# maxjiang93/space_time_pde

Hardware: AMD Instinct MI355X
Metric: query-points/sec (fwd+PDE-residual bwd), rb2d 128^3 latent (higher is better)
Workload: dtype f32; 1 GPU; BASELINE configs[1]: latent [1,32,128,128,32], 2^20 query points, RB2 (3 transport + continuity), ImNet nf=32 softplus, L1 losses, backward to ImNet + UNet3d parameters; points=1048576, parallelism=points sharded x1, unet=UNet3d(igres=(32, 128, 128), nf=16, mf=256) fwd+bwd inside the timed step

## Files before the change

include/stpde_hip.h:

```cpp
#ifndef STPDE_HIP_H
#define STPDE_HIP_H

#ifdef __cplusplus
extern "C" {
#endif

#define STPDE_OK 0
#define STPDE_E_BADARG 1
#define STPDE_E_UNSUPPORTED 2
#define STPDE_E_LAUNCH 3

#define STPDE_ACT_TANH 0
#define STPDE_ACT_RELU 1
#define STPDE_ACT_SOFTPLUS 2
#define STPDE_ACT_ELU 3
#define STPDE_ACT_SWISH 4
#define STPDE_ACT_LEAKYRELU 5

#define STPDE_XT 3
#define STPDE_PBAR_SLOTS 64

typedef struct {
  int S1;
  int S2;
// ... 2 lines not shown
  int act;
  float act_param;
  int combo;
  float alpha[6];
} stpde_jet_cfg;

int stpde_version(void);
int stpde_last_error(char* buf, unsigned long n);
#define STPDE_TUNE_CONV3_LDS_OFF 0
#define STPDE_TUNE_CONV3_LDS_MINBLK 1
#define STPDE_TUNE_CONV3_LDS_GX 2
#define STPDE_TUNE_CONV_WGRAD_LDS_GX 3
#define STPDE_TUNE_CONV1_WGRAD_LDS_GX 4
#define STPDE_TUNE_WGRAD_FP32_SWAP 5
#define STPDE_TUNE_FC2_BWD_FUSED 6
#define STPDE_TUNE_COUNT 7
int stpde_tune(const char* name, int value);
int stpde_trace_enable(int on);
long stpde_trace_read(char* buf, unsigned long n);

typedef struct {
  int P, N, B, n0, n1, n2, C;
  int p_base;
  float lo_c[3], hi_c[3], cube[3];
  float alpha[6];
} stpde_gather_desc;
int stpde_lig_gather(const stpde_gather_desc* d, const float* pts, const float* latent, float* X, float* XR,
                     float* coef, int* cell, float* cw , void* stream);

typedef struct {
  int ntiles, KT, MT, first_hidden;
// ... 30 lines not shown

int stpde_jet_layer_bwd_to(const stpde_layer_desc* d, const float* abar_out, const float* WhT_pack, const float* in_pre,
                           float* abar_in, const float* cw, float* act_param_bar, const void* WhT_pack_bf16, void* stream);

int stpde_jet_wgrad(const stpde_layer_desc* d, int SP, const float* abar_out, const float* in_pre, const float* X,
                    const float* tanc0, float* dW_aug, const float* cw, void* stream);

int stpde_jet_fc1_bwd_supported(const stpde_layer_desc* d);
int stpde_jet_fc1_bwd(const stpde_layer_desc* d, const float* abar1, const void* WhT_pack_bf16, const float* z0,
                      const float* tanc0, const float* cw, const float* X, float* abar0, float* abar0_tan, float* dW_aug,
                      float* act_param_bar, void* stream);

int stpde_jet_fc2_bwd_supported(const stpde_layer_desc* d);
int stpde_jet_fc2_bwd(const stpde_layer_desc* d, const float* abar2, const float* WhT_pack, const float* pre1, const float* X,
                      const float* cw, float* abar1, float* dW_aug, float* act_param_bar, void* stream);

int stpde_lig_reduce_fwd(const stpde_jet_cfg* cfg, int S_mlp, int P, int n_out, const float* out_pre,
                         const float* coef, float* jets, long ldp, void* stream);
int stpde_lig_reduce_bwd(const stpde_jet_cfg* cfg, int S_mlp, int P, int n_out, const float* jets_bar, long ldp,
                         const float* coef, float* abar_out, void* stream);

int stpde_jet_tan0_reduce(int ntiles, int MT, const float* abar0_tan, float* dW_aug, int ldw, int det ,
                          void* stream);

typedef struct {
  int ntiles, nlayers, C, n1, n2;
  int MT[8];
  int SP[8];
  int packed[8];
  int S[8];
// ... 40 lines not shown
  unsigned long sort_tmp_bytes;
  float* abar4x;
} stpde_lig_workspace;
#define STPDE_F_STASH 1
#define STPDE_F_VALUE_TILES 2
#define STPDE_F_FUSED_TAIL 4
#define STPDE_F_TAN0_ROWSUM 8
#define STPDE_F_DETERMINISTIC 16
#define STPDE_F_WGRAD 32
#define STPDE_F_WGRAD_FP32 64
#define STPDE_F_PHASE_A 128
#define STPDE_F_PHASE_B 256
#define STPDE_F_NO_FC1_FUSED 512
#define STPDE_F_DET 1024
#define STPDE_F_FC2_FUSED 2048
int stpde_lig_imnet_jet_fwd(const stpde_imnet_plan* plan, const stpde_jet_cfg* cfg_mlp, const stpde_jet_cfg* cfg_out,
                            const stpde_gather_desc* gd, const float* pts, const float* latent,
                            const stpde_lig_workspace* ws, float* jets, long ldp, int flags, void* stream);
int stpde_lig_imnet_jet_bwd(const stpde_imnet_plan* plan, const stpde_jet_cfg* cfg_mlp, const stpde_jet_cfg* cfg_out,
                            const stpde_jet_cfg* cfg_val, const stpde_gather_desc* gd, const stpde_lig_workspace* ws,
                            const float* jets_bar, long ldp, float* dW_flat, float* dlatent, float* act_param_bar,
                            int flags, void* stream);
unsigned long stpde_lig_sort_tmp_bytes(int P, long n_nodes);
int stpde_lig_cell_sort(int P, long n_nodes, const int* cell, int* perm, int* start, void* tmp, unsigned long tmp_bytes,
                        void* stream);

typedef struct {
  int P, N, B, dim, C;
  int n[4];
  float lo_c[4], hi_c[4], cube[4];
// ... 256 lines not shown
```

space_time_pde_amd/_lib.py:

```python
import ctypes as C
import os
import subprocess
import threading

_HERE = os.path.dirname(os.path.abspath(__file__))
_CSRC = os.path.join(_HERE, "csrc")
LIB_PATH = os.environ.get("STPDE_LIB") or os.path.join(_HERE, "libstpde_hip.so")
_SOURCES = ["jet_layer.hip", "jet_layer_s00.hip", "jet_layer_s03.hip", "jet_layer_s30.hip", "jet_layer_s31.hip", "jet_layer_s32.hip", "jet_layer_s34.hip", "jet_layer_s36.hip", "jet_tail.hip", "jet_wgrad.hip", "jet_wgrad_s00.hip", "jet_wgrad_s30.hip", "jet_wgrad_s31.hip", "jet_wgrad_s32.hip", "jet_wgrad_s34.hip", "jet_wgrad_s36.hip", "jet_fc1_bwd.hip", "jet_fc2_bwd.hip", "lig_gather_reduce.hip", "lig_pipeline.hip", "interp_nd.hip", "conv3d.hip", "conv3d_fused.hip", "optim.hip", "residual.hip", "bn.hip", "resample.hip", "sampler.hip", "sampler_median.hip", "api.cpp"]
_HIPFLAGS = ["--offload-arch=gfx950", "-O3", "-std=c++17", "-fPIC", "-ffp-contract=off", "-munsafe-fp-atomics",
             "--offload-compress"]

ABI_VERSION = 316

ACT_CODES = {"tanh": 0, "relu": 1, "softplus": 2, "elu": 3, "swish": 4, "leakyrelu": 5}
PBAR_SLOTS = 64
XT = 3


class JetCfg(C.Structure):
    _fields_ = [("S1", C.c_int), ("S2", C.c_int), ("pair0", C.c_int * 6), ("pair1", C.c_int * 6),
                ("act", C.c_int), ("act_param", C.c_float), ("combo", C.c_int), ("alpha", C.c_float * 6)]


class GatherDesc(C.Structure):
# ... 21 lines not shown
class ImNetPlanDesc(C.Structure):
    _fields_ = [("nlayers", C.c_int), ("cin", C.c_int), ("cout", C.c_int), ("nf16", C.c_int), ("KT", C.c_int * 8),
                ("MT", C.c_int * 8), ("Wh", C.c_void_p * 8), ("WhT", C.c_void_p * 8), ("Ws", C.c_void_p * 8),
                ("WsL", C.c_void_p * 8), ("tanc", C.c_void_p * 8), ("Wh16", C.c_void_p * 8), ("WhT16", C.c_void_p * 8),
                ("mfma_bf16", C.c_int), ("packed_mask", C.c_int), ("dw_off", C.c_long * 8)]


class LigWorkspace(C.Structure):
    _fields_ = [("X", C.c_void_p), ("XR", C.c_void_p), ("coef", C.c_void_p), ("cw", C.c_void_p), ("cell", C.c_void_p),
                ("pre", C.c_void_p * 8), ("abar2x", C.c_void_p), ("abar3x", C.c_void_p), ("tan0", C.c_void_p),
                ("abar0", C.c_void_p), ("abar1x", C.c_void_p), ("abar0x", C.c_void_p), ("xrows", C.c_void_p), ("perm", C.c_void_p), ("start", C.c_void_p),
                ("sort_tmp", C.c_void_p), ("sort_tmp_bytes", C.c_ulong), ("abar4x", C.c_void_p)]


F_STASH, F_VALUE_TILES, F_FUSED_TAIL, F_TAN0_ROWSUM, F_DETERMINISTIC, F_WGRAD, F_WGRAD_FP32 = 1, 2, 4, 8, 16, 32, 64
F_PHASE_A, F_PHASE_B, F_NO_FC1_FUSED, F_DET, F_FC2_FUSED = 128, 256, 512, 1024, 2048
LOSS_DET = 16


class Conv3dDesc(C.Structure):
    _fields_ = [("B", C.c_int), ("T", C.c_int), ("Z", C.c_int), ("X", C.c_int), ("Ci", C.c_int), ("Co", C.c_int),
                ("ksize", C.c_int), ("det", C.c_int), ("mfma_bf16", C.c_int)]


class Conv3dFusedArgs(C.Structure):
    _fields_ = [("d", Conv3dDesc), ("x", C.c_void_p), ("w_pack", C.c_void_p), ("bias", C.c_void_p), ("y", C.c_void_p),
                ("x2", C.c_void_p), ("w2_pack", C.c_void_p), ("y2", C.c_void_p), ("wo2_pack", C.c_void_p),
                ("bias2", C.c_void_p), ("in_sums", C.c_void_p), ("in_gamma", C.c_void_p), ("in_beta", C.c_void_p),
                ("in_running_mean", C.c_void_p), ("in_running_var", C.c_void_p), ("in_stat", C.c_void_p),
                ("out_sums", C.c_void_p), ("m", C.c_void_p), ("m_stat", C.c_void_p), ("m_gamma", C.c_void_p),
                ("m_beta", C.c_void_p), ("m_bsum", C.c_void_p), ("Ci2", C.c_int), ("Co2", C.c_int),
# ... 173 lines not shown
    "stpde_jet_layer_bwd_to": ([C.POINTER(LayerDesc)] + [_VP] * 8, C.c_int),
    "stpde_jet_tail_fwd": ([C.POINTER(JetCfg), C.c_int, C.c_int, _VP, _VP, C.POINTER(_VP), C.POINTER(_VP), C.POINTER(_VP),
                            C.POINTER(_VP), _VP, _VP], C.c_int),
    "stpde_jet_tail_bwd": ([C.POINTER(JetCfg), C.c_int, C.c_int, _VP, C.POINTER(_VP), C.POINTER(_VP), C.POINTER(_VP), _VP,
                            _VP, _VP], C.c_int),
    "stpde_jet_tail_fwd_p": ([C.POINTER(JetCfg), C.c_int, C.c_int, _VP, _VP, C.POINTER(_VP), C.POINTER(_VP), C.POINTER(_VP),
                              C.POINTER(_VP), _VP, C.c_int, C.POINTER(_VP), _VP], C.c_int),
    "stpde_jet_tail_bwd_p": ([C.POINTER(JetCfg), C.c_int, C.c_int, _VP, C.POINTER(_VP), C.POINTER(_VP), C.POINTER(_VP), _VP,
                              _VP, C.c_int, C.POINTER(_VP), _VP], C.c_int),
    "stpde_jet_tan0_reduce": ([C.c_int, C.c_int, _VP, _VP, C.c_int, C.c_int, _VP], C.c_int),
    "stpde_jet_wgrad": ([C.POINTER(LayerDesc), C.c_int] + [_VP] * 7, C.c_int),
    "stpde_jet_fc1_bwd_supported": ([C.POINTER(LayerDesc)], C.c_int),
    "stpde_jet_fc1_bwd": ([C.POINTER(LayerDesc)] + [_VP] * 11, C.c_int),
    "stpde_jet_fc2_bwd_supported": ([C.POINTER(LayerDesc)], C.c_int),
    "stpde_jet_fc2_bwd": ([C.POINTER(LayerDesc)] + [_VP] * 9, C.c_int),
    "stpde_lig_reduce_fwd": ([C.POINTER(JetCfg), C.c_int, C.c_int, C.c_int, _VP, _VP, _VP, C.c_long, _VP], C.c_int),
    "stpde_lig_reduce_bwd": ([C.POINTER(JetCfg), C.c_int, C.c_int, C.c_int, _VP, C.c_long, _VP, _VP, _VP], C.c_int),
    "stpde_lig_xbar_scatter": ([C.POINTER(XbarDesc), C.POINTER(_VP), C.POINTER(_VP), _VP, _VP, _VP], C.c_int),
    "stpde_lig_xbar_rows": ([C.POINTER(XbarDesc), C.POINTER(_VP), C.POINTER(_VP), _VP, _VP], C.c_int),
    "stpde_lig_dlatent_reduce": ([C.c_int] * 5 + [_VP] * 5, C.c_int),
    "stpde_lig_imnet_jet_fwd": ([C.POINTER(ImNetPlanDesc), C.POINTER(JetCfg), C.POINTER(JetCfg), C.POINTER(GatherDesc), _VP,
                                 _VP, C.POINTER(LigWorkspace), _VP, C.c_long, C.c_int, _VP], C.c_int),
    "stpde_lig_imnet_jet_bwd": ([C.POINTER(ImNetPlanDesc), C.POINTER(JetCfg), C.POINTER(JetCfg), C.POINTER(JetCfg),
                                 C.POINTER(GatherDesc), C.POINTER(LigWorkspace), _VP, C.c_long, _VP, _VP, _VP, C.c_int, _VP],
                                C.c_int),
    "stpde_lig_sort_tmp_bytes": ([C.c_int, C.c_long], C.c_ulong),
    "stpde_lig_cell_sort": ([C.c_int, C.c_long, _VP, _VP, _VP, _VP, C.c_ulong, _VP], C.c_int),
    "stpde_interp_fwd": ([C.POINTER(InterpDesc)] + [_VP] * 7, C.c_int),
    "stpde_interp_bwd_grid": ([C.POINTER(InterpDesc)] + [_VP] * 5, C.c_int),
    "stpde_conv3d_fwd": ([C.POINTER(Conv3dDesc)] + [_VP] * 5, C.c_int),
# ... 170 lines not shown
```

space_time_pde_amd/csrc/api.cpp:

```cpp
#include <hip/hip_runtime.h>

#include <cstdarg>
#include <cstdio>
#include <cstring>
#include <mutex>
#include <set>
#include <string>

#include "../../include/stpde_hip.h"

static thread_local char g_err[512] = "";

void stpde_set_error(const char* fmt, ...) {
  va_list ap;
  va_start(ap, fmt);
  vsnprintf(g_err, sizeof(g_err), fmt, ap);
  va_end(ap);
}

int stpde_check_launch(const char* what) {
  hipError_t e = hipGetLastError();
  if (e != hipSuccess) {
    stpde_set_error("%s: launch failed: %s", what, hipGetErrorString(e));
    return STPDE_E_LAUNCH;
  }
  return STPDE_OK;
}

extern "C" int stpde_version(void) { return 316; }

#include <atomic>
static const char* const g_tune_names[STPDE_TUNE_COUNT] = {"conv3_lds_off", "conv3_lds_minblk", "conv3_lds_gx", "conv_wgrad_lds_gx",
                                                           "conv1_wgrad_lds_gx", "wgrad_fp32_swap", "fc2_bwd_fused"};
static std::atomic<int> g_tune[STPDE_TUNE_COUNT];
int stpde_tune_get(int key) { return (key >= 0 && key < STPDE_TUNE_COUNT) ? g_tune[key].load(std::memory_order_relaxed) : 0; }
extern "C" int stpde_tune(const char* name, int value) {
  if (!name) return -1;
  for (int k = 0; k < STPDE_TUNE_COUNT; ++k)
    if (!strcmp(name, g_tune_names[k])) return g_tune[k].exchange(value);
  stpde_set_error("stpde_tune: unknown key '%s'", name);
  return -1;
}

extern "C" int stpde_last_error(char* buf, unsigned long n) {
  if (!buf || n == 0) return STPDE_E_BADARG;
  strncpy(buf, g_err, n - 1);
  buf[n - 1] = 0;
  return STPDE_OK;
// ... 29 lines not shown
```

space_time_pde_amd/csrc/lig_pipeline.hip:

```cpp
#include <hipcub/hipcub.hpp>

#include "common.h"

namespace {

struct Seq {
  int rc = STPDE_OK;
  template <class F>
  void operator()(F&& f) {
    if (rc == STPDE_OK) rc = f();
  }
};

bool is_packed(const stpde_imnet_plan* p, int l) { return l >= 0 && ((p->packed_mask >> l) & 1); }

int packed_flags(const stpde_imnet_plan* p, int l, int writes) {
  return ((l >= 2 && is_packed(p, l - 1)) ? 1 : 0) | ((writes >= 0 && is_packed(p, writes)) ? 2 : 0) | (is_packed(p, l) ? 4 : 0);
}

stpde_layer_desc layer_desc(int ntiles, const stpde_imnet_plan* p, int l, const stpde_jet_cfg& cfg, int bf16) {
  stpde_layer_desc d{};
  d.ntiles = ntiles;
  d.KT = p->KT[l];
  d.MT = p->MT[l];
// ... 94 lines not shown
      const float* Wh[3] = {p->Wh[3], p->Wh[4], p->Wh[5]};
      const float* Wsk[3] = {p->Ws[3], p->Ws[4], p->Ws[5]};
      const float* tc[3] = {p->tanc[3], p->tanc[4], p->tanc[5]};
      float* outs[3] = {ws->pre[3], ws->pre[4], ws->pre[5]};
      seq([&] {
        const void* w16[3] = {p->Wh16[3], p->Wh16[4], p->Wh16[5]};
        const bool pk = is_packed(p, 2);
        return stpde_jet_tail_fwd_p(&lcfg, lnt, p->nf16, prev, ws->X, Wh, Wsk, tc, outs, ws->cw, pk ? 3 : 0, pk ? w16 : nullptr,
                                    stream);
      });
      break;
    }
    const void* w16 = p->mfma_bf16 ? p->Wh16[l] : nullptr;
    stpde_layer_desc d = layer_desc(lnt, p, l, lcfg, w16 ? p->mfma_bf16 : 0);
    d.packed = packed_flags(p, l, l) & 3;
    seq([&] {
      return stpde_jet_layer_fwd(&d, prev, ws->X, p->Wh[l], p->Ws[l], p->tanc[l], p->Ws[0], p->tanc[0], ws->pre[l], ws->cw, w16,
                                 (l == 1 && stash) ? ws->pre[0] : nullptr, stream);
    });
    prev = ws->pre[l];
  }
  seq([&] { return stpde_lig_reduce_fwd(cfg_out, S, gd->P, p->cout, ws->pre[NL - 1], ws->coef, jets, ldp, stream); });
  return seq.rc;
}

extern "C" int stpde_lig_imnet_jet_bwd(const stpde_imnet_plan* p, const stpde_jet_cfg* cfg_mlp, const stpde_jet_cfg* cfg_out,
                                       const stpde_jet_cfg* cfg_val, const stpde_gather_desc* gd, const stpde_lig_workspace* ws,
                                       const float* jets_bar, long ldp, float* dW_flat, float* dlatent, float* act_param_bar,
                                       int flags, void* stream) {
  if (!p || !cfg_mlp || !cfg_out || !cfg_val || !gd || !ws || !jets_bar || p->nlayers != 6 || (gd->P & 1) || !ws->pre[0]) {
    stpde_set_error("lig_imnet_jet_bwd: bad argument (needs the stash of a forward call with STPDE_F_STASH)");
    return STPDE_E_BADARG;
// ... 67 lines not shown
      const bool pk = is_packed(p, 2);
      return stpde_jet_tail_bwd_p(&cfg, nt, p->nf16, ws->pre[5], WhT, pre, outs, ws->cw, act_param_bar, pk ? 3 : 0,
                                  pk ? w16 : nullptr, stream);
    });
  };
  auto dgrad_l = [&](int l) {
    const void* w16 = p->mfma_bf16 ? p->WhT16[l] : nullptr;
    stpde_layer_desc d = layer_desc(nt, p, l, cfg, w16 ? p->mfma_bf16 : 0);
    d.packed = packed_flags(p, l, l - 1);
    if (l > 1 && abar[l - 1] != ws->pre[l - 1]) {
      seq([&] {
        return stpde_jet_layer_bwd_to(&d, abar[l], p->WhT[l], ws->pre[l - 1], abar[l - 1], ws->cw, act_param_bar, w16, stream);
      });
      return;
    }
    seq([&] {
      return stpde_jet_layer_bwd(&d, abar[l], p->WhT[l], l > 1 ? ws->pre[l - 1] : nullptr, ws->X, p->Ws[0], p->tanc[0], abar0,
                                 ws->cw, act_param_bar, w16, (l == 1 && split0) ? ws->tan0 : nullptr, l == 1 ? z0 : nullptr,
                                 stream);
    });
  };
  const bool fc1_fused_on = [&]() -> bool {
    if (!wgrad || !split0 || (flags & STPDE_F_NO_FC1_FUSED)) return false;
    stpde_layer_desc d = layer_desc(nt, p, 1, cfg, p->mfma_bf16 ? p->mfma_bf16 : 0);
    d.packed = packed_flags(p, 1, 0);
    return p->WhT16[1] && stpde_jet_fc1_bwd_supported(&d) != 0 && abar0 != z0;
  }();
  auto fc1_fused_ok = [&]() -> bool { return fc1_fused_on; };
  auto fc1_fused = [&] {
    stpde_layer_desc d = layer_desc(nt, p, 1, cfg, p->mfma_bf16);
    d.packed = packed_flags(p, 1, 0);
    d.det = det;
// ... 89 lines not shown
```

space_time_pde_amd/lig_jet.py:

```python
import ctypes as C
import dataclasses
import math
import os
import threading

import numpy as np
import torch

from . import _lib
from ._lib import XT, GatherDesc, GatherNdDesc, ImNetPlanDesc, JetCfg, LayerDesc, LigWorkspace, XbarDesc, check, ptr, stream_ptr

_FRAG = 256
MAX_LATENT_CHANNELS = 16 * (XT - 1) + 4 - 3 - 1
MAX_AUG_FEATURES = 16 * (XT - 1) + 4
ND_VALUE_DIMS = (1, 2, 4)
ND_TRAIN_MAX_CHANNELS = 32

nd_backward = os.getenv("STPDE_ND_BACKWARD", "0").strip().lower() not in ("", "0", "false", "no", "off")


def set_nd_backward(on):
    global nd_backward
    prev, nd_backward = nd_backward, bool(on)
    return prev
# ... 309 lines not shown
    hi_c: list
    cube: list
    P_pad: int
    budget: object
    recompute: bool
    chunk: int
    need_grad: bool
    det: bool
    det_dlatent: bool
    value_tiles: bool
    tan0_rowsum: bool
    wgrad_split: bool
    fused_tail: bool
    fc1_fused: bool
    fc2_fused: bool
    nd_backward: bool
    nd_jets: bool
    nd_jet_backward: bool
    pipeline: bool
    tail: bool
    SP0: int
    split0: bool
    mult: int

    @classmethod
    def make(cls, plan, act, act_param, first, pairs, combo, precision, grid_shape, box, budget=None, B=1, N=0,
             chunk_points=None, need_grad=True):
        precision = precision or mlp_precision
        if precision not in ("fp32", "bf16", "fp32x3"):
            raise ValueError("mlp precision must be 'fp32', 'bf16' or 'fp32x3'")
# ... 5 lines not shown
        if act in ("relu", "leakyrelu") and ppairs:
            cfg, S, _ = make_cfg(act, act_param, True, [])
        tail = _tail_applies(fused_tail, plan.nf, cfg, cfg_out.combo)
        packed = (precision == "bf16" and packed_stash and plan.nf == 32 and S <= 6 and tail and cfg.S1 == 3 and tan0_rowsum)
        mult = (8 if S == 1 else 2) if dim == 3 else 4 * (16 >> dim)
        chunk_points = chunk_points or (DEFAULT_CHUNK if dim == 3 else (DEFAULT_CHUNK // 2) * (16 >> dim))
        P, SP0 = B * N, 1 + cfg.S1
        return cls(plan=plan, cfg=cfg, cfg_out=cfg_out, cfg_val=make_cfg(act, act_param, False, [])[0], S=S, S_out=S_out,
                   pairs=ppairs, bf16=precision in ("bf16", "fp32x3"), nsplit=3 if precision == "fp32x3" else 1,
                   packed_mask=31 if packed else 0, B=B, N=N, grid_shape=tuple(grid_shape), lo_c=box[0], hi_c=box[1],
                   cube=box[2], P_pad=P + ((-P) % mult if dim == 3 else 0),
                   budget=budget if budget is not None else memory_budget, recompute=bool(force_recompute),
                   chunk=max(mult, chunk_points // mult * mult), need_grad=bool(need_grad), det=bool(_lib.deterministic),
                   det_dlatent=bool(deterministic_dlatent), value_tiles=bool(value_tiles), tan0_rowsum=bool(tan0_rowsum),
                   wgrad_split=bool(wgrad_split), fused_tail=bool(fused_tail), fc1_fused=fc1_fused_enabled(),
                   fc2_fused=fc2_fused_enabled(),
                   nd_backward=bool(nd_backward), nd_jets=bool(nd_jets),
                   nd_jet_backward=bool(nd_jets and nd_jet_backward),
                   pipeline=bool(use_pipeline and profile is None and dim == 3),
                   tail=tail, SP0=SP0, split0=bool(SP0 == 4 and tan0_rowsum), mult=mult)

    def plan_chunk(self, points):
        object.__setattr__(self, "chunk", points)


def _AW(call):
    return 2 * _lib.DET_K if call.det else 1


def _dw_slice(call, dw_flat, l):
    off, mp, ka = call.plan.dw_off[l]
# ... 58 lines not shown
    gd = GatherDesc()
    gd.P, gd.N, gd.B = Pc, call.N, call.B
    gd.n0, gd.n1, gd.n2, gd.C = latent.shape[1], latent.shape[2], latent.shape[3], latent.shape[4]
    for k in range(3):
        gd.lo_c[k], gd.hi_c[k], gd.cube[k] = call.lo_c[k], call.hi_c[k], call.cube[k]
    gd.p_base = p0
    for k in range(6):
        gd.alpha[k] = call.cfg_out.alpha[k]
    return gd


def _flags(call, need_grad, need_wgrad=True):
    bits = ((need_grad, _lib.F_STASH), (call.value_tiles, _lib.F_VALUE_TILES), (call.fused_tail, _lib.F_FUSED_TAIL),
            (call.tan0_rowsum, _lib.F_TAN0_ROWSUM), (call.det_dlatent, _lib.F_DETERMINISTIC), (need_wgrad, _lib.F_WGRAD),
            (not call.wgrad_split, _lib.F_WGRAD_FP32), (not call.fc1_fused, _lib.F_NO_FC1_FUSED), (call.det, _lib.F_DET),
            (call.fc2_fused, _lib.F_FC2_FUSED))
    return sum(bit for on, bit in bits if on)


def nd_tiles(P, dim):
    tp = 16 >> dim
    return (-(-P // tp) + 3) // 4 * 4


_LAYER_BUFS = tuple("buf%d" % l for l in range(1, 6))
_FWD_ORDER = {True: ("X", "cw", "coef", "cell") + _LAYER_BUFS + ("z0",),
              False: ("X", "cw", "roww", "coef", "cell", "buf1", "z0") + _LAYER_BUFS[1:]}
_BWD_ORDER = {True: ("abar2x", "abar3x", "abar1x", "abar4x", "abar0x", "tan0", "abar0"),
              False: ("abar0", "abar0x", "tan0", "abar1x", "abar4x", "abar3x", "abar2x")}
_DTYPES = dict(cell=torch.int32, perm=torch.int32, start=torch.int32, sort_tmp=torch.uint8)
SORT_TMP_PLAN_BYTES = 24
# ... 131 lines not shown
    for l in range(1, 6):
        lay = plan.layers[l]
        if tail and l == 3:
            arr = lambda ts: (C.c_void_p * 3)(*[t.data_ptr() for t in ts])
            pk_tail = (call.packed_mask >> 2) & 1
            w16s = arr([packs16[(k, "Wh")] for k in (3, 4, 5)]) if pk_tail else None
            with _timed("tail_fwd"):
                check(L.stpde_jet_tail_fwd_p(C.byref(lcfg), lnt, plan.nf // 16, ptr(bufs[2]), ptr(X),
                                             arr([pv(packs, k, "Wh") for k in (3, 4, 5)]),
                                             arr([pv(packs, k, "Ws") for k in (3, 4, 5)]),
                                             arr([pv(packs, k, "tanc") for k in (3, 4, 5)]), arr(bufs[3:6]), ptr(cw),
                                             3 if pk_tail else 0, w16s, st))
            break
        w16 = packs16.get((l, "Wh")) if packs16 else None
        d = _layer_desc(call, lnt, lay, lcfg, l == 1, call.nsplit if w16 is not None else 0, _pk(call, l, l) & 3)
        with _timed("layer%d_fwd" % l):
            check(L.stpde_jet_layer_fwd(C.byref(d), ptr(bufs[l - 1]), ptr(X), ptr(pv(packs, l, "Wh")),
                                        ptr(pv(packs, l, "Ws")), ptr(pv(packs, l, "tanc")), ptr(pv(packs, 0, "Ws")),
                                        ptr(pv(packs, 0, "tanc")), ptr(bufs[l]), ptr(cw), ptr(w16),
                                        ptr(z0) if l == 1 else None, st))
    if nd_jet:
        with _timed("reduce_nd_jet"):
            check(L.stpde_lig_reduce_nd_jet_fwd(C.byref(call.cfg_out), S, plan.dim, Pc, nt, plan.cout, ptr(bufs[5]), ptr(coef),
                                                C.c_void_p(jets.data_ptr() + 4 * p0), jets.shape[2], st))
    elif nd:
        with _timed("reduce_nd"):
            check(L.stpde_lig_reduce_nd_fwd(plan.dim, Pc, nt, plan.cout, ptr(bufs[5]), ptr(roww),
                                            C.c_void_p(jets.data_ptr() + 4 * p0), jets.shape[2], st))
    else:
        with _timed("reduce_fwd"):
            check(L.stpde_lig_reduce_fwd(C.byref(call.cfg_out), S, Pc, plan.cout, ptr(bufs[5]), ptr(coef),
                                         C.c_void_p(jets.data_ptr() + 4 * p0), jets.shape[2], st))
# ... 67 lines not shown
                arr = lambda ts: (C.c_void_p * 3)(*[t.data_ptr() for t in ts])
                pk_tail = (call.packed_mask >> 2) & 1
                w16s = (C.c_void_p * 3)(packs16[(3, "WhT")].data_ptr(), packs16[(4, "WhT")].data_ptr(), None) \
                    if pk_tail else None
                with _timed("tail_dgrad"):
                    check(L.stpde_jet_tail_bwd_p(C.byref(cfg), nt, plan.nf // 16, ptr(bufs[5]),
                                                 arr([pv(packs, k, "WhT") for k in (3, 4, 5)]),
                                                 arr([bufs[2], bufs[3], bufs[4]]), arr([abar[2], abar[3], abar[4]]),
                                                 ptr(cw), ptr(pbar), 3 if pk_tail else 0, w16s, st))
            continue
        if l > 1 and abar[l - 1] is not bufs[l - 1]:
            with _timed("layer%d_dgrad" % l):
                check(L.stpde_jet_layer_bwd_to(C.byref(d), ptr(abar[l]), ptr(pv(packs, l, "WhT")), ptr(bufs[l - 1]),
                                               ptr(abar[l - 1]), ptr(cw), ptr(pbar), ptr(w16), st))
            continue
        with _timed("layer%d_dgrad" % l):
            check(L.stpde_jet_layer_bwd(C.byref(d), ptr(abar[l]), ptr(pv(packs, l, "WhT")),
                                        ptr(bufs[l - 1]) if l > 1 else None, ptr(X), ptr(pv(packs, 0, "Ws")),
                                        ptr(pv(packs, 0, "tanc")), ptr(abar0), ptr(cw), ptr(pbar), ptr(w16),
                                        ptr(tan0) if l == 1 else None, ptr(z0) if l == 1 else None, st))
    if need_wgrad:
        lay = plan.layers[0]
        d = _layer_desc(call, nt, lay, cfg, False, call.packed_mask & 1, _pk(call, 0, -1) & 4)
        dw0 = _dw_slice(call, dw_flat, 0)
        with _timed("layer0_wgrad"):
            if split0:
                d.cfg = call.cfg_val
                check(L.stpde_jet_wgrad(C.byref(d), 1, ptr(abar0), None, ptr(X), None, ptr(dw0), None, st))
                if nd_jet:
                    check(L.stpde_jet_tan0_reduce_nd(nt, MT0, ptr(tan0), ptr(dw0), plan.dw_off[0][2], int(call.det), plan.dim, st))
                else:
                    check(L.stpde_jet_tan0_reduce(nt, MT0, ptr(tan0), ptr(dw0), plan.dw_off[0][2], int(call.det), st))
# ... 235 lines not shown
packed_stash = True
fused_tail = True

force_recompute = False


def fc1_fused_enabled():
    return os.environ.get("STPDE_FC1_FUSED", "1") != "0"


fc2_fused = None


def fc2_fused_enabled():
    return bool(fc2_fused) and _lib.tune_value("fc2_bwd_fused") != 2


DEFAULT_CHUNK = 1 << 20

mlp_precision = os.environ.get("STPDE_MLP_PRECISION", "fp32")


def set_mlp_precision(precision):
    global mlp_precision
    if precision not in ("fp32", "bf16", "fp32x3"):
        raise ValueError("mlp precision must be 'fp32', 'bf16' or 'fp32x3'")
    prev, mlp_precision = mlp_precision, precision
    return prev


# ... 81 lines not shown
```

space_time_pde_amd/train_step.py:

```python
import os

import torch
import torch.distributed as dist
import torch.nn.functional as F

from . import _lib, lig_jet
from .local_implicit_grid import query_local_implicit_grid


last_collectives = []


class _SumGradAcrossRanks(torch.autograd.Function):

    @staticmethod
    def forward(ctx, x):
        return x.view_as(x)

    @staticmethod
    def backward(ctx, g):
        hooks = lig_jet.sync_hooks
        done = hooks.get("dlatent_done") if hooks else None
        if done is None:
            g = g.contiguous()
# ... 63 lines not shown
def sharded_step(unet, imnet, pde_layer, input_grid, point_coord, point_value, n_points_global, alpha_reg=1.0,
                 alpha_pde=1.0, loss_type="l1", xmin=0.0, xmax=1.0, distributed=None, sync_unet_grads=False):
    if distributed is None:
        distributed = dist.is_available() and dist.is_initialized() and dist.get_world_size() > 1
    if loss_type not in _LOSS_SUMS:
        raise KeyError(loss_type)
    if distributed and any(t.requires_grad and not t.is_leaf for t in (getattr(pde_layer, "params", None) or {}).values()):
        raise NotImplementedError("sharded_step(distributed=True): a grad-requiring equation coefficient must be a leaf tensor "
                                  "(the gradient of a leaf behind it would not be summed over ranks)")
    prev_deferred = getattr(unet, "deferred_weight_grads", None)
    if prev_deferred is not None:
        unet.deferred_weight_grads = os.environ.get("STPDE_UNET_DEFERRED", "1") != "0"
    prev_fc2 = lig_jet.fc2_fused
    if prev_fc2 is None:
        lig_jet.fc2_fused = True
    try:
        return _sharded_step(unet, imnet, pde_layer, input_grid, point_coord, point_value, n_points_global, alpha_reg,
                             alpha_pde, loss_type, xmin, xmax, distributed, sync_unet_grads)
    finally:
        lig_jet.fc2_fused = prev_fc2
        if prev_deferred is not None:
            unet.deferred_weight_grads = prev_deferred


def _sharded_step(unet, imnet, pde_layer, input_grid, point_coord, point_value, n_points_global, alpha_reg, alpha_pde,
                  loss_type, xmin, xmax, distributed, sync_unet_grads):
    latent_grid = unet(input_grid).permute(0, 2, 3, 4, 1)
    if distributed:
        latent_grid = _SumGradAcrossRanks.apply(latent_grid)
    pde_layer.update_forward_method(lambda pts: query_local_implicit_grid(imnet, latent_grid, pts, xmin, xmax))
    overlap_sync = distributed and os.environ.get("STPDE_OVERLAP_SYNC", "1") != "0"
    lig_jet.expect_two_phase = bool(overlap_sync)
    try:
        pred, residues = pde_layer(point_coord, return_residue=True)
    finally:
# ... 186 lines not shown
```

Measured before the change: 2.572 million query-points/s.

## Add two-team staggered fc1 forward and dgrad kernel for overlap

Adds a new kernel for the first hidden layer, forward and input-gradient. Each 512-thread block runs two teams of four waves that process alternate tiles on a fixed barrier schedule, offset by half a unit, so one team's MFMA work can overlap the other's loads and epilogue. It is enabled by default inside the sharded train step when the layer shape is supported, and can be tuned off. The cost is a more complex fixed barrier schedule, a larger LDS ring, and a layout that holds only for KT=32 and MT=16 in fp32.

New measurement: 2.554 million query-points/s. About the same (-0.7%).

```diff
diff --git a/include/stpde_hip.h b/include/stpde_hip.h
--- a/include/stpde_hip.h
+++ b/include/stpde_hip.h
@@ -40,7 +40,8 @@
 #define STPDE_TUNE_CONV1_WGRAD_LDS_GX 4
 #define STPDE_TUNE_WGRAD_FP32_SWAP 5
 #define STPDE_TUNE_FC2_BWD_FUSED 6
-#define STPDE_TUNE_COUNT 7
+#define STPDE_TUNE_FC1_DUO 7
+#define STPDE_TUNE_COUNT 8
 int stpde_tune(const char* name, int value);
 int stpde_trace_enable(int on);
 long stpde_trace_read(char* buf, unsigned long n);
@@ -101,6 +102,15 @@
 int stpde_jet_fc2_bwd_supported(const stpde_layer_desc* d);
 int stpde_jet_fc2_bwd(const stpde_layer_desc* d, const float* abar2, const float* WhT_pack, const float* pre1, const float* X,
                       const float* cw, float* abar1, float* dW_aug, float* act_param_bar, void* stream);
+
+int stpde_jet_fc1_duo_supported(const stpde_layer_desc* d);
+int stpde_jet_fc1_duo_schedule(int kind, int nunits, int grid, int block, int* out);
+int stpde_jet_fc1_duo_fwd(const stpde_layer_desc* d, const float* in_pre, const float* X, const float* Wh_pack,
+                          const float* Ws_pack, const float* tanc, const float* W0s_pack, const float* tanc0, float* out_pre,
+                          const float* cw, const void* Wh_pack_bf16, float* z0, void* stream);
+int stpde_jet_fc1_duo_bwd(const stpde_layer_desc* d, const float* abar_out, const float* WhT_pack, float* in_pre, const float* X,
+                          const float* W0s_pack, const float* tanc0, float* abar0, const float* cw, float* act_param_bar,
+                          const void* WhT_pack_bf16, float* abar0_tan, const float* z0, void* stream);
 
 int stpde_lig_reduce_fwd(const stpde_jet_cfg* cfg, int S_mlp, int P, int n_out, const float* out_pre,
                          const float* coef, float* jets, long ldp, void* stream);
@@ -171,6 +181,7 @@
 #define STPDE_F_NO_FC1_FUSED 512
 #define STPDE_F_DET 1024
 #define STPDE_F_FC2_FUSED 2048
+#define STPDE_F_FC1_DUO 4096
 int stpde_lig_imnet_jet_fwd(const stpde_imnet_plan* plan, const stpde_jet_cfg* cfg_mlp, const stpde_jet_cfg* cfg_out,
                             const stpde_gather_desc* gd, const float* pts, const float* latent,
                             const stpde_lig_workspace* ws, float* jets, long ldp, int flags, void* stream);
diff --git a/space_time_pde_amd/_lib.py b/space_time_pde_amd/_lib.py
--- a/space_time_pde_amd/_lib.py
+++ b/space_time_pde_amd/_lib.py
@@ -6,7 +6,7 @@
 _HERE = os.path.dirname(os.path.abspath(__file__))
 _CSRC = os.path.join(_HERE, "csrc")
 LIB_PATH = os.environ.get("STPDE_LIB") or os.path.join(_HERE, "libstpde_hip.so")
-_SOURCES = ["jet_layer.hip", "jet_layer_s00.hip", "jet_layer_s03.hip", "jet_layer_s30.hip", "jet_layer_s31.hip", "jet_layer_s32.hip", "jet_layer_s34.hip", "jet_layer_s36.hip", "jet_tail.hip", "jet_wgrad.hip", "jet_wgrad_s00.hip", "jet_wgrad_s30.hip", "jet_wgrad_s31.hip", "jet_wgrad_s32.hip", "jet_wgrad_s34.hip", "jet_wgrad_s36.hip", "jet_fc1_bwd.hip", "jet_fc2_bwd.hip", "lig_gather_reduce.hip", "lig_pipeline.hip", "interp_nd.hip", "conv3d.hip", "conv3d_fused.hip", "optim.hip", "residual.hip", "bn.hip", "resample.hip", "sampler.hip", "sampler_median.hip", "api.cpp"]
+_SOURCES = ["jet_layer.hip", "jet_layer_s00.hip", "jet_layer_s03.hip", "jet_layer_s30.hip", "jet_layer_s31.hip", "jet_layer_s32.hip", "jet_layer_s34.hip", "jet_layer_s36.hip", "jet_tail.hip", "jet_wgrad.hip", "jet_wgrad_s00.hip", "jet_wgrad_s30.hip", "jet_wgrad_s31.hip", "jet_wgrad_s32.hip", "jet_wgrad_s34.hip", "jet_wgrad_s36.hip", "jet_fc1_bwd.hip", "jet_fc2_bwd.hip", "jet_fc1_duo.hip", "lig_gather_reduce.hip", "lig_pipeline.hip", "interp_nd.hip", "conv3d.hip", "conv3d_fused.hip", "optim.hip", "residual.hip", "bn.hip", "resample.hip", "sampler.hip", "sampler_median.hip", "api.cpp"]
 _HIPFLAGS = ["--offload-arch=gfx950", "-O3", "-std=c++17", "-fPIC", "-ffp-contract=off", "-munsafe-fp-atomics",
              "--offload-compress"]
 
@@ -59,7 +59,7 @@
 
 
 F_STASH, F_VALUE_TILES, F_FUSED_TAIL, F_TAN0_ROWSUM, F_DETERMINISTIC, F_WGRAD, F_WGRAD_FP32 = 1, 2, 4, 8, 16, 32, 64
-F_PHASE_A, F_PHASE_B, F_NO_FC1_FUSED, F_DET, F_FC2_FUSED = 128, 256, 512, 1024, 2048
+F_PHASE_A, F_PHASE_B, F_NO_FC1_FUSED, F_DET, F_FC2_FUSED, F_FC1_DUO = 128, 256, 512, 1024, 2048, 4096
 LOSS_DET = 16
 
 
@@ -263,6 +263,10 @@
     "stpde_jet_fc1_bwd": ([C.POINTER(LayerDesc)] + [_VP] * 11, C.c_int),
     "stpde_jet_fc2_bwd_supported": ([C.POINTER(LayerDesc)], C.c_int),
     "stpde_jet_fc2_bwd": ([C.POINTER(LayerDesc)] + [_VP] * 9, C.c_int),
+    "stpde_jet_fc1_duo_supported": ([C.POINTER(LayerDesc)], C.c_int),
+    "stpde_jet_fc1_duo_schedule": ([C.c_int, C.c_int, C.c_int, C.c_int, C.POINTER(C.c_int)], C.c_int),
+    "stpde_jet_fc1_duo_fwd": ([C.POINTER(LayerDesc)] + [_VP] * 12, C.c_int),
+    "stpde_jet_fc1_duo_bwd": ([C.POINTER(LayerDesc)] + [_VP] * 13, C.c_int),
     "stpde_lig_reduce_fwd": ([C.POINTER(JetCfg), C.c_int, C.c_int, C.c_int, _VP, _VP, _VP, C.c_long, _VP], C.c_int),
     "stpde_lig_reduce_bwd": ([C.POINTER(JetCfg), C.c_int, C.c_int, C.c_int, _VP, C.c_long, _VP, _VP, _VP], C.c_int),
     "stpde_lig_xbar_scatter": ([C.POINTER(XbarDesc), C.POINTER(_VP), C.POINTER(_VP), _VP, _VP, _VP], C.c_int),
diff --git a/space_time_pde_amd/csrc/api.cpp b/space_time_pde_amd/csrc/api.cpp
--- a/space_time_pde_amd/csrc/api.cpp
+++ b/space_time_pde_amd/csrc/api.cpp
@@ -31,7 +31,8 @@
 
 #include <atomic>
 static const char* const g_tune_names[STPDE_TUNE_COUNT] = {"conv3_lds_off", "conv3_lds_minblk", "conv3_lds_gx", "conv_wgrad_lds_gx",
-                                                           "conv1_wgrad_lds_gx", "wgrad_fp32_swap", "fc2_bwd_fused"};
+                                                           "conv1_wgrad_lds_gx", "wgrad_fp32_swap", "fc2_bwd_fused",
+                                                           "fc1_duo"};
 static std::atomic<int> g_tune[STPDE_TUNE_COUNT];
 int stpde_tune_get(int key) { return (key >= 0 && key < STPDE_TUNE_COUNT) ? g_tune[key].load(std::memory_order_relaxed) : 0; }
 extern "C" int stpde_tune(const char* name, int value) {
diff --git a/space_time_pde_amd/csrc/jet_fc1_duo.hip b/space_time_pde_amd/csrc/jet_fc1_duo.hip
--- /dev/null
+++ b/space_time_pde_amd/csrc/jet_fc1_duo.hip
@@ -0,0 +1,318 @@
+#include "jet_layer_impl.h"
+
+#define DUO_BARRIER()                                      \
+  do {                                                     \
+    asm volatile("s_waitcnt lgkmcnt(0)" ::: "memory");     \
+    __builtin_amdgcn_s_barrier();                          \
+    asm volatile("" ::: "memory");                         \
+  } while (0)
+
+enum { DUO_FWD = 0, DUO_DGRAD = 1 };
+
+struct DuoSched {
+  int NB;
+  int OFF;
+  int first[2];
+  int stride;
+  int n[2];
+  int pre[2];
+  int post[2];
+  int total;
+};
+
+__host__ __device__ inline DuoSched duo_schedule(int kind, int nunits, int grid, int block) {
+  DuoSched s;
+  s.NB = kind == DUO_FWD ? 2 + 8 : 1 + 4 + 3;
+  s.OFF = s.NB / 2;
+  s.stride = 2 * grid;
+  for (int t = 0; t < 2; ++t) {
+    s.first[t] = 2 * block + t;
+    s.n[t] = s.first[t] < nunits ? (nunits - s.first[t] + s.stride - 1) / s.stride : 0;
+  }
+  const int nmax = s.n[0] > s.n[1] ? s.n[0] : s.n[1];
+  s.total = s.OFF + s.NB * nmax;
+  s.pre[0] = 0;
+  s.pre[1] = s.OFF;
+  for (int t = 0; t < 2; ++t) s.post[t] = s.total - s.pre[t] - s.NB * s.n[t];
+  return s;
+}
+
+template <int S1, int S2, int PRO, int EPI, int ACT>
+__global__ __launch_bounds__(512, 2) void k_layer_duo(LayerArgs a, int nunits) {
+  constexpr int S = 1 + S1 + S2, NW = 4, MCg = 4, GK = 4;
+  constexpr bool FWD = EPI == EPI_FWD;
+  static_assert((PRO == PRO_L0 && EPI == EPI_FWD) || (PRO == PRO_NONE && EPI == EPI_ADJ_L0), "fc1's forward or input gradient");
+  static_assert(S1 == 3 && S <= 5, "tangent streams, at most five streams");
+  constexpr int KT = FWD ? 32 : 16, MT = FWD ? 16 : 32, NG = KT / GK;
+  __shared__ __attribute__((aligned(16))) float ring[2][2][GK][S][256];
+  const int lane = threadIdx.x & 63;
+  const int wave = __builtin_amdgcn_readfirstlane(threadIdx.x >> 6);
+  const int team = wave >> 2, wv = wave & 3;
+  float (*hb)[GK][S][256] = ring[team];
+  const int lo = lane * 4;
+  const DuoSched sc = duo_schedule(FWD ? DUO_FWD : DUO_DGRAD, nunits, gridDim.x, blockIdx.x);
+  const int npre = team ? sc.pre[1] : sc.pre[0], npost = team ? sc.post[1] : sc.post[0];
+  const int nmine = team ? sc.n[1] : sc.n[0], ufirst = team ? sc.first[1] : sc.first[0], ustride = sc.stride;
+  float pacc = 0.f;
+
+#pragma unroll 1
+  for (int i = 0; i < npre; ++i) DUO_BARRIER();
+#pragma unroll 1
+  for (int un = 0; un < nmine; ++un) {
+    const int u = ufirst + un * ustride;
+    if constexpr (FWD) DUO_BARRIER();
+    const int tile = FWD ? u : (u >> 1);
+    const int pass0 = FWD ? 0 : (u & 1);
+    float cq[6];
+    load_cq<S2>(a.cw, tile * 2 + ((lane & 15) >> 3), cq);
+    f32x4 xb[1][XT];
+    if (PRO == PRO_L0 || EPI == EPI_FWD) {
+#pragma unroll
+      for (int xt = 0; xt < XT; ++xt) xb[0][xt] = ld4x(a.X + ((size_t)tile * XT + xt) * 256 + lo, xt);
+    }
+    const auto z0r = opt_store_rsrc(a.Z0 ? a.Z0 + (size_t)tile * KT * 256 : nullptr, (unsigned)KT * 1024u);
+
+    auto produce = [&](int kt, int buf, int slot) {
+      f32x4 raw[S], B[S];
+      if (PRO == PRO_L0) {
+        raw[0] = layer0_block(a.W0s, KT, kt, lo, xb[0]);
+        opt_st4(z0r, kt * 1024 + lane * 16, raw[0]);
+#pragma unroll
+        for (int d = 0; d < 3; ++d) raw[1 + d] = ld4(a.tanc0 + ((size_t)d * KT + kt) * 256 + lo);
+#pragma unroll
+        for (int p = 0; p < S2; ++p) raw[4 + p] = f32x4{0.f, 0.f, 0.f, 0.f};
+        act_jet_fwd<S1, S2, ACT>(a.cfg, raw, B, cq);
+      } else {
+#pragma unroll
+        for (int st = 0; st < S; ++st) B[st] = ld4(a.Bin + (((size_t)tile * S + st) * KT + kt) * 256 + lo);
+      }
+#pragma unroll
+      for (int st = 0; st < S; ++st) st4(&hb[buf][slot][st][lo], B[st]);
+    };
+    auto store_block = [&](const f32x4* B, int buf, int slot) {
+#pragma unroll
+      for (int st = 0; st < S; ++st) st4(&hb[buf][slot][st][lo], B[st]);
+    };
+
+    int mt0 = (pass0 * NW + wv) * MCg;
+    asm volatile("" : "+s"(mt0));
+    f32x4 acc[MCg][S];
+#pragma unroll
+    for (int mi = 0; mi < MCg; ++mi)
+#pragma unroll
+      for (int st = 0; st < S; ++st) acc[mi][st] = f32x4{0.f, 0.f, 0.f, 0.f};
+    f32x4 z0p[FWD ? 1 : MCg];
+    if constexpr (!FWD) {
+#pragma unroll
+      for (int mi = 0; mi < MCg; ++mi) z0p[mi] = ld4(a.Z0 + ((size_t)tile * MT + mt0 + mi) * 256 + lo);
+    }
+    const float* wp = a.Wp + (size_t)mt0 * 256 + lo;
+    f32x4 wr[4][MCg];
+#pragma unroll
+    for (int q = 0; q < 3; ++q)
+#pragma unroll
+      for (int mi = 0; mi < MCg; ++mi) wr[q][mi] = ld4(wp + ((size_t)q * MT + mi) * 256);
+    produce(wv, 0, wv);
+    DUO_BARRIER();
+#pragma unroll 1
+    for (int gi = 0; gi < NG; ++gi) {
+      const int buf = gi & 1;
+      const int gnext = gi + 1 < NG ? gi + 1 : gi;
+      f32x4 rawn[FWD ? 1 : S];
+      if constexpr (!FWD) {
+#pragma unroll
+        for (int st = 0; st < S; ++st) rawn[st] = ld4(a.Bin + (((size_t)tile * S + st) * KT + GK * gnext + wv) * 256 + lo);
+      }
+      f32x4 w0n[FWD ? XT : 1], tcn[FWD ? 3 : 1];
+      if constexpr (FWD) {
+        const int kt = GK * gnext + wv;
+#pragma unroll
+        for (int xt = 0; xt < XT; ++xt) w0n[xt] = ld4x(a.W0s + ((size_t)xt * KT + kt) * 256 + lo, xt);
+#pragma unroll
+        for (int d = 0; d < 3; ++d) tcn[d] = ld4(a.tanc0 + ((size_t)d * KT + kt) * 256 + lo);
+      }
+#pragma unroll
+      for (int q = 0; q < 4; ++q) {
+        const int kt = 4 * gi + q;
+        const int ktn = kt + 3 < KT ? kt + 3 : KT - 1;
+        f32x4 B[S];
+#pragma unroll
+        for (int st = 0; st < S; ++st) B[st] = ld4(&hb[buf][q][st][lo]);
+#pragma unroll
+        for (int mi = 0; mi < MCg; ++mi)
+#pragma unroll
+          for (int r = 0; r < 4; ++r)
+#pragma unroll
+            for (int st = 0; st < S; ++st) acc[mi][st] = mfma4(wr[q][mi][r], B[st][r], acc[mi][st]);
+#pragma unroll
+        for (int mi = 0; mi < MCg; ++mi) wr[(q + 3) & 3][mi] = ld4(wp + ((size_t)ktn * MT + mi) * 256);
+      }
+      if constexpr (!FWD) {
+        store_block(rawn, buf ^ 1, wv);
+      } else {
+        const int kt = GK * gnext + wv;
+        f32x4 raw[S], B[S], part[XT];
+#pragma unroll
+        for (int xt = 0; xt < XT; ++xt) {
+          f32x4 c = f32x4{0.f, 0.f, 0.f, 0.f};
+#pragma unroll
+          for (int r = 0; r < x_live(xt); ++r) c = mfma4(w0n[xt][r], xb[0][xt][r], c);
+          part[xt] = c;
+        }
+        raw[0] = (part[0] + part[1]) + part[2];
+        opt_st4(z0r, kt * 1024 + lane * 16, raw[0]);
+#pragma unroll
+        for (int d = 0; d < 3; ++d) raw[1 + d] = tcn[d];
+#pragma unroll
+        for (int p = 0; p < S2; ++p) raw[4 + p] = f32x4{0.f, 0.f, 0.f, 0.f};
+        act_jet_fwd<S1, S2, ACT>(a.cfg, raw, B, cq);
+        store_block(B, buf ^ 1, wv);
+      }
+      DUO_BARRIER();
+    }
+    if constexpr (!FWD) {
+      f32x4 tcl[MCg][3];
+#pragma unroll
+      for (int mi = 0; mi < MCg; ++mi)
+#pragma unroll
+        for (int d = 0; d < 3; ++d) tcl[mi][d] = ld4(a.tanc0 + ((size_t)d * MT + mt0 + mi) * 256 + lo);
+      __builtin_amdgcn_sched_barrier(0);
+#pragma unroll
+      for (int mi = 0; mi < MCg; ++mi) {
+        layer_epilogue<S1, S2, EPI, ACT, 0>(a, tile, mt0 + mi, MT, lane, acc[mi], xb, cq, pacc, &z0p[mi], nullptr, nullptr, tcl[mi]);
+        if (mi + 1 < MCg) DUO_BARRIER();
+      }
+    } else {
+      f32x4 wsc[XT], tcc[3], wsn[XT], tcn2[3];
+      auto fetch = [&](int mt, f32x4* w, f32x4* t) {
+#pragma unroll
+        for (int xt = 0; xt < XT; ++xt) w[xt] = ld4x(a.Wsp + ((size_t)xt * MT + mt) * 256 + lo, xt);
+#pragma unroll
+        for (int d = 0; d < 3; ++d) t[d] = ld4(a.tanc + ((size_t)d * MT + mt) * 256 + lo);
+      };
+      fetch(mt0, wsc, tcc);
+#pragma unroll
+      for (int mi = 0; mi < MCg; ++mi) {
+        if (mi + 1 < MCg) fetch(mt0 + mi + 1, wsn, tcn2);
+        __builtin_amdgcn_sched_barrier(0);
+        layer_epilogue<S1, S2, EPI, ACT, 0>(a, tile, mt0 + mi, MT, lane, acc[mi], xb, cq, pacc, nullptr, nullptr, wsc, tcc);
+#pragma unroll
+        for (int xt = 0; xt < XT; ++xt) wsc[xt] = wsn[xt];
+#pragma unroll
+        for (int d = 0; d < 3; ++d) tcc[d] = tcn2[d];
+      }
+    }
+  }
+#pragma unroll 1
+  for (int i = 0; i < npost; ++i) DUO_BARRIER();
+  flush_pbar<EPI, ACT>(a, pacc, lane);
+}
+
+template <int S1, int S2, int PRO, int EPI, int ACT>
+static int launch_duo(const LayerArgs& a, hipStream_t stream) {
+  const int nunits = EPI == EPI_FWD ? a.ntiles : 2 * a.ntiles;
+  int gx = 256;
+  if (gx > (nunits + 1) / 2) gx = (nunits + 1) / 2;
+  STPDE_LAUNCH((k_layer_duo<S1, S2, PRO, EPI, ACT>), dim3(gx), dim3(512), 0, stream, a, nunits);
+  return stpde_check_launch("k_layer_duo");
+}
+
+template <int S1, int S2, int PRO, int EPI>
+static int launch_duo_act(const LayerArgs& a, hipStream_t stream) {
+  constexpr bool PWL = !(EPI == EPI_FWD && S2 == 1);
+  switch (a.cfg.act) {
+    case STPDE_ACT_TANH: return launch_duo<S1, S2, PRO, EPI, STPDE_ACT_TANH>(a, stream);
+    case STPDE_ACT_RELU: return launch_duo<S1, S2, PRO, EPI, PWL ? STPDE_ACT_RELU : STPDE_ACT_TANH>(a, stream);
+    case STPDE_ACT_SOFTPLUS: return launch_duo<S1, S2, PRO, EPI, STPDE_ACT_SOFTPLUS>(a, stream);
+    case STPDE_ACT_ELU: return launch_duo<S1, S2, PRO, EPI, STPDE_ACT_ELU>(a, stream);
+    case STPDE_ACT_LEAKYRELU: return launch_duo<S1, S2, PRO, EPI, PWL ? STPDE_ACT_LEAKYRELU : STPDE_ACT_TANH>(a, stream);
+    default: return launch_duo<S1, S2, PRO, EPI, STPDE_ACT_SWISH>(a, stream);
+  }
+}
+
+extern "C" int stpde_jet_fc1_duo_supported(const stpde_layer_desc* d) {
+  if (!d) return 0;
+  const bool combo = d->cfg.S2 == 1 && d->cfg.combo;
+  const bool both = d->first_hidden && d->mfma_bf16 == 0 && d->packed == 0 && d->KT == 32 && d->MT == 16 && d->ntiles > 0 &&
+                    d->ntiles < (1 << 29) && d->cfg.S1 == 3 && (d->cfg.S2 == 0 || combo) && d->cfg.act >= 0 && d->cfg.act <= 5;
+  if (!both) return 0;
+  const bool pwl = d->cfg.act == STPDE_ACT_RELU || d->cfg.act == STPDE_ACT_LEAKYRELU;
+  return (combo && pwl) ? 2 : 3;
+}
+
+extern "C" int stpde_jet_fc1_duo_schedule(int kind, int nunits, int grid, int block, int* out) {
+  if ((kind != DUO_FWD && kind != DUO_DGRAD) || nunits < 0 || grid < 1 || block < 0 || block >= grid || !out) {
+    stpde_set_error("jet_fc1_duo_schedule: bad argument");
+    return STPDE_E_BADARG;
+  }
+  const DuoSched s = duo_schedule(kind, nunits, grid, block);
+  const int v[12] = {s.NB, s.OFF, s.first[0], s.first[1], s.stride, s.n[0], s.n[1], s.pre[0], s.pre[1], s.post[0], s.post[1], s.total};
+  for (int i = 0; i < 12; ++i) out[i] = v[i];
+  return STPDE_OK;
+}
+
+static int duo_refuse() {
+  stpde_set_error("jet_fc1_duo: exact fp32, unpacked buffers, first hidden layer of the reference width only (KT = 32, MT = 16, "
+                  "S1 = 3, S2 = 0 or the combined stream; see stpde_jet_fc1_duo_supported)");
+  return STPDE_E_UNSUPPORTED;
+}
+
+extern "C" int stpde_jet_fc1_duo_fwd(const stpde_layer_desc* d, const float* in_pre, const float* X, const float* Wh_pack,
+                                     const float* Ws_pack, const float* tanc, const float* W0s_pack, const float* tanc0,
+                                     float* out_pre, const float* cw, const void* Wh_pack_bf16, float* z0, void* stream) {
+  (void)in_pre;
+  (void)Wh_pack_bf16;
+  if (!(stpde_jet_fc1_duo_supported(d) & 1)) return duo_refuse();
+  if (!X || !Wh_pack || !Ws_pack || !tanc || !W0s_pack || !tanc0 || !out_pre || (d->cfg.S2 && !cw)) {
+    stpde_set_error("jet_fc1_duo_fwd: null pointer");
+    return STPDE_E_BADARG;
+  }
+  LayerArgs a{};
+  a.Wp = Wh_pack;
+  a.X = X;
+  a.W0s = W0s_pack;
+  a.tanc0 = tanc0;
+  a.Wsp = Ws_pack;
+  a.tanc = tanc;
+  a.Out = out_pre;
+  a.cw = cw;
+  a.nsplit = 1;
+  a.KT = d->KT;
+  a.MT = d->MT;
+  a.ntiles = d->ntiles;
+  a.cfg = d->cfg;
+  a.Z0 = z0;
+  if (d->cfg.S2 == 1) return launch_duo_act<3, 1, PRO_L0, EPI_FWD>(a, (hipStream_t)stream);
+  return launch_duo_act<3, 0, PRO_L0, EPI_FWD>(a, (hipStream_t)stream);
+}
+
+extern "C" int stpde_jet_fc1_duo_bwd(const stpde_layer_desc* d, const float* abar_out, const float* WhT_pack, float* in_pre,
+                                     const float* X, const float* W0s_pack, const float* tanc0, float* abar0, const float* cw,
+                                     float* act_param_bar, const void* WhT_pack_bf16, float* abar0_tan, const float* z0,
+                                     void* stream) {
+  (void)in_pre;
+  (void)X;
+  (void)W0s_pack;
+  (void)WhT_pack_bf16;
+  if (!(stpde_jet_fc1_duo_supported(d) & 2)) return duo_refuse();
+  if (!abar_out || !WhT_pack || !tanc0 || !abar0 || !z0 || (d->cfg.S2 && !cw) || (z0 == abar0 && !abar0_tan)) {
+    stpde_set_error("jet_fc1_duo_bwd: null pointer (z0 may alias abar0 only when abar0 holds the value stream alone)");
+    return STPDE_E_BADARG;
+  }
+  LayerArgs a{};
+  a.Bin = abar_out;
+  a.Wp = WhT_pack;
+  a.tanc0 = tanc0;
+  a.cw = cw;
+  a.pbar = act_param_bar;
+  a.nsplit = 1;
+  a.KT = d->MT;
+  a.MT = d->KT;
+  a.ntiles = d->ntiles;
+  a.cfg = d->cfg;
+  a.Out = abar0;
+  a.Tan0 = abar0_tan;
+  a.Z0 = const_cast<float*>(z0);
+  if (d->cfg.S2 == 1) return launch_duo_act<3, 1, PRO_NONE, EPI_ADJ_L0>(a, (hipStream_t)stream);
+  return launch_duo_act<3, 0, PRO_NONE, EPI_ADJ_L0>(a, (hipStream_t)stream);
+}
diff --git a/space_time_pde_amd/csrc/lig_pipeline.hip b/space_time_pde_amd/csrc/lig_pipeline.hip
--- a/space_time_pde_amd/csrc/lig_pipeline.hip
+++ b/space_time_pde_amd/csrc/lig_pipeline.hip
@@ -132,8 +132,10 @@
     const void* w16 = p->mfma_bf16 ? p->Wh16[l] : nullptr;
     stpde_layer_desc d = layer_desc(lnt, p, l, lcfg, w16 ? p->mfma_bf16 : 0);
     d.packed = packed_flags(p, l, l) & 3;
-    seq([&] {
-      return stpde_jet_layer_fwd(&d, prev, ws->X, p->Wh[l], p->Ws[l], p->tanc[l], p->Ws[0], p->tanc[0], ws->pre[l], ws->cw, w16,
+    const int duo = stpde_tune_get(STPDE_TUNE_FC1_DUO);
+    const bool duo_on = l == 1 && (flags & STPDE_F_FC1_DUO) && duo != 2 && duo != 4 && (stpde_jet_fc1_duo_supported(&d) & 1);
+    seq([&] {
+      return (duo_on ? stpde_jet_fc1_duo_fwd : stpde_jet_layer_fwd)(&d, prev, ws->X, p->Wh[l], p->Ws[l], p->tanc[l], p->Ws[0], p->tanc[0], ws->pre[l], ws->cw, w16,
                                  (l == 1 && stash) ? ws->pre[0] : nullptr, stream);
     });
     prev = ws->pre[l];
@@ -231,8 +233,10 @@
       });
       return;
     }
-    seq([&] {
-      return stpde_jet_layer_bwd(&d, abar[l], p->WhT[l], l > 1 ? ws->pre[l - 1] : nullptr, ws->X, p->Ws[0], p->tanc[0], abar0,
+    const int duo = stpde_tune_get(STPDE_TUNE_FC1_DUO);
+    const bool duo_on = l == 1 && !dfirst && (flags & STPDE_F_FC1_DUO) && duo != 2 && duo != 3 && (stpde_jet_fc1_duo_supported(&d) & 2);
+    seq([&] {
+      return (duo_on ? stpde_jet_fc1_duo_bwd : stpde_jet_layer_bwd)(&d, abar[l], p->WhT[l], l > 1 ? ws->pre[l - 1] : nullptr, ws->X, p->Ws[0], p->tanc[0], abar0,
                                  ws->cw, act_param_bar, w16, (l == 1 && split0) ? ws->tan0 : nullptr, l == 1 ? z0 : nullptr,
                                  stream);
     });
diff --git a/space_time_pde_amd/lig_jet.py b/space_time_pde_amd/lig_jet.py
--- a/space_time_pde_amd/lig_jet.py
+++ b/space_time_pde_amd/lig_jet.py
@@ -347,6 +347,7 @@
     fused_tail: bool
     fc1_fused: bool
     fc2_fused: bool
+    fc1_duo: int
     nd_backward: bool
     nd_jets: bool
     nd_jet_backward: bool
@@ -382,7 +383,7 @@
                    chunk=max(mult, chunk_points // mult * mult), need_grad=bool(need_grad), det=bool(_lib.deterministic),
                    det_dlatent=bool(deterministic_dlatent), value_tiles=bool(value_tiles), tan0_rowsum=bool(tan0_rowsum),
                    wgrad_split=bool(wgrad_split), fused_tail=bool(fused_tail), fc1_fused=fc1_fused_enabled(),
-                   fc2_fused=fc2_fused_enabled(),
+                   fc2_fused=fc2_fused_enabled(), fc1_duo=fc1_duo_enabled(),
                    nd_backward=bool(nd_backward), nd_jets=bool(nd_jets),
                    nd_jet_backward=bool(nd_jets and nd_jet_backward),
                    pipeline=bool(use_pipeline and profile is None and dim == 3),
@@ -471,7 +472,7 @@
     bits = ((need_grad, _lib.F_STASH), (call.value_tiles, _lib.F_VALUE_TILES), (call.fused_tail, _lib.F_FUSED_TAIL),
             (call.tan0_rowsum, _lib.F_TAN0_ROWSUM), (call.det_dlatent, _lib.F_DETERMINISTIC), (need_wgrad, _lib.F_WGRAD),
             (not call.wgrad_split, _lib.F_WGRAD_FP32), (not call.fc1_fused, _lib.F_NO_FC1_FUSED), (call.det, _lib.F_DET),
-            (call.fc2_fused, _lib.F_FC2_FUSED))
+            (call.fc2_fused, _lib.F_FC2_FUSED), (call.fc1_duo, _lib.F_FC1_DUO))
     return sum(bit for on, bit in bits if on)
 
 
@@ -633,8 +634,9 @@
             break
         w16 = packs16.get((l, "Wh")) if packs16 else None
         d = _layer_desc(call, lnt, lay, lcfg, l == 1, call.nsplit if w16 is not None else 0, _pk(call, l, l) & 3)
+        duo = l == 1 and (call.fc1_duo & 1) and (L.stpde_jet_fc1_duo_supported(C.byref(d)) & 1)
         with _timed("layer%d_fwd" % l):
-            check(L.stpde_jet_layer_fwd(C.byref(d), ptr(bufs[l - 1]), ptr(X), ptr(pv(packs, l, "Wh")),
+            check((L.stpde_jet_fc1_duo_fwd if duo else L.stpde_jet_layer_fwd)(C.byref(d), ptr(bufs[l - 1]), ptr(X), ptr(pv(packs, l, "Wh")),
                                         ptr(pv(packs, l, "Ws")), ptr(pv(packs, l, "tanc")), ptr(pv(packs, 0, "Ws")),
                                         ptr(pv(packs, 0, "tanc")), ptr(bufs[l]), ptr(cw), ptr(w16),
                                         ptr(z0) if l == 1 else None, st))
@@ -732,8 +734,9 @@
                 check(L.stpde_jet_layer_bwd_to(C.byref(d), ptr(abar[l]), ptr(pv(packs, l, "WhT")), ptr(bufs[l - 1]),
                                                ptr(abar[l - 1]), ptr(cw), ptr(pbar), ptr(w16), st))
             continue
+        duo = l == 1 and (call.fc1_duo & 2) and (L.stpde_jet_fc1_duo_supported(C.byref(d)) & 2)
         with _timed("layer%d_dgrad" % l):
-            check(L.stpde_jet_layer_bwd(C.byref(d), ptr(abar[l]), ptr(pv(packs, l, "WhT")),
+            check((L.stpde_jet_fc1_duo_bwd if duo else L.stpde_jet_layer_bwd)(C.byref(d), ptr(abar[l]), ptr(pv(packs, l, "WhT")),
                                         ptr(bufs[l - 1]) if l > 1 else None, ptr(X), ptr(pv(packs, 0, "Ws")),
                                         ptr(pv(packs, 0, "tanc")), ptr(abar0), ptr(cw), ptr(pbar), ptr(w16),
                                         ptr(tan0) if l == 1 else None, ptr(z0) if l == 1 else None, st))
@@ -999,6 +1002,13 @@
 
 def fc2_fused_enabled():
     return bool(fc2_fused) and _lib.tune_value("fc2_bwd_fused") != 2
+
+
+fc1_duo = None
+
+
+def fc1_duo_enabled():
+    return {0: 3, 1: 3, 2: 0, 3: 1, 4: 2}.get(_lib.tune_value("fc1_duo"), 3) if fc1_duo else 0
 
 
 DEFAULT_CHUNK = 1 << 20
diff --git a/space_time_pde_amd/train_step.py b/space_time_pde_amd/train_step.py
--- a/space_time_pde_amd/train_step.py
+++ b/space_time_pde_amd/train_step.py
@@ -101,11 +101,15 @@
     prev_fc2 = lig_jet.fc2_fused
     if prev_fc2 is None:
         lig_jet.fc2_fused = True
+    prev_duo = lig_jet.fc1_duo
+    if prev_duo is None:
+        lig_jet.fc1_duo = True
     try:
         return _sharded_step(unet, imnet, pde_layer, input_grid, point_coord, point_value, n_points_global, alpha_reg,
                              alpha_pde, loss_type, xmin, xmax, distributed, sync_unet_grads)
     finally:
         lig_jet.fc2_fused = prev_fc2
+        lig_jet.fc1_duo = prev_duo
         if prev_deferred is not None:
             unet.deferred_weight_grads = prev_deferred
 
```
